# shenweichen/DeepCTR

Hardware: NVIDIA H100
Metric: samples/sec fwd+bwd DeepFM Criteo-synth (higher is better)
Workload: dtype f32

## Files before the change

deepctr_b200/_lib.py:

```python
import ctypes as C
import os
import subprocess

_HERE = os.path.dirname(os.path.abspath(__file__))
LIB_PATH = os.path.join(_HERE, "libb2ctr.so")
CSRC = os.path.join(_HERE, "csrc")

OK, ERR_INVALID_ARG, ERR_CUDA, ERR_UNSUPPORTED, ERR_WORKSPACE = 0, -1, -2, -3, -4
IDX_I32, IDX_I64 = 0, 1
POOL_NONE, POOL_SUM, POOL_MEAN, POOL_MAX = 0, 1, 2, 3
MASK_NONE, MASK_ZERO_ID, MASK_LENGTH = 0, 1, 2
HASH_NONE, HASH_FARM, HASH_FARM_MASK_ZERO = 0, 1, 2
WEIGHT_NONE, WEIGHT_RAW, WEIGHT_SOFTMAX = 0, 1, 2
ACT_NONE, ACT_RELU, ACT_SIGMOID, ACT_TANH = 0, 1, 2, 3
GEMM_FP32, GEMM_BF16X3 = 0, 1
TASK_BINARY, TASK_REGRESSION = 0, 1
MAX_FEATURES = 128
UNIFORM_STORE_GRADS = 1

ACT_BY_NAME = {None: ACT_NONE, "linear": ACT_NONE, "relu": ACT_RELU, "sigmoid": ACT_SIGMOID,
               "tanh": ACT_TANH}
POOL_BY_NAME = {"sum": POOL_SUM, "mean": POOL_MEAN, "max": POOL_MAX}


# ... 50 lines not shown
                ("dk", C.c_void_p), ("lddk", C.c_int64), ("dv", C.c_void_p), ("lddv", C.c_int64)]


_vp, _i32, _i64, _f32, _sz, _u64 = C.c_void_p, C.c_int32, C.c_int64, C.c_float, C.c_size_t, C.c_uint64

SIGNATURES = {
    "b2ctr_abi_version": (_i32, []),
    "b2ctr_last_error": (C.c_char_p, []),
    "b2ctr_launch_count": (_i64, []),
    "b2ctr_reset_launch_count": (None, []),
    "b2ctr_embed_gather_fwd": (_i32, [C.POINTER(Feature), _i32, _i64, _vp]),
    "b2ctr_embed_scatter_add": (_i32, [C.POINTER(Feature), _i32, _i64, _f32, _vp]),
    "b2ctr_embed_gather_uniform_fwd": (_i32, [C.POINTER(UniformGather), _i64, _vp]),
    "b2ctr_embed_scatter_uniform_bwd": (_i32, [C.POINTER(UniformGather), _vp, _vp, _vp, _f32, _f32,
                                               _i64, _vp]),
    "b2ctr_embed_oob_count": (_i32, [C.POINTER(C.c_int64), _i32, _vp]),
    "b2ctr_embed_update_sorted_workspace_bytes": (_sz, [_i32, _i32, _i64]),
    "b2ctr_embed_update_sorted": (_i32, [C.POINTER(UniformGather), _vp, _vp, _vp, _i32, _f32, _f32, _f32,
                                         C.POINTER(C.c_void_p), C.POINTER(C.c_void_p), _i64, _vp, _sz, _vp]),
    "b2ctr_hash64": (_i32, [_vp, _i32, _i64, _i64, _i32, _vp, _vp]),
    "b2ctr_init_normal": (_i32, [_vp, _i64, _f32, _f32, _u64, _vp]),
    "b2ctr_gemm_workspace_bytes": (_sz, [C.POINTER(Gemm)]),
    "b2ctr_enable_peer_access": (_i32, [_i32]),
    "b2ctr_host_pack": (_i32, [C.POINTER(C.c_void_p), C.POINTER(C.c_int64), C.POINTER(C.c_int64), _i32, _vp, _i32]),
    "b2ctr_gemm": (_i32, [C.POINTER(Gemm), _vp, _sz, _vp]),
    "b2ctr_planes_bytes": (_sz, [_i64, _i64]),
    "b2ctr_split_planes": (_i32, [_vp, _i64, _i64, _i64, _vp, _vp]),
    "b2ctr_bias_act_bwd_workspace_bytes": (_sz, [_i64, _i64]),
    "b2ctr_bias_act_bwd": (_i32, [_vp, _vp, _vp, _vp, _i64, _i64, _i64, _i32, _vp, _sz, _vp]),
    "b2ctr_bias_act_bwd_planes": (_i32, [_vp, _vp, _vp, _vp, _vp, _i64, _i64, _i64, _i32, _vp, _sz, _vp]),
# ... 157 lines not shown
```

deepctr_b200/csrc/common.cuh:

```cuda
#pragma once
#include <cuda_runtime.h>
#include <stdint.h>
#include <stdio.h>
#include <atomic>
#include "../../include/b2ctr.h"

namespace b2ctr {

void set_error(const char* fmt, ...);
extern std::atomic<long long> g_launches;
inline void count_launch(int n = 1) { g_launches.fetch_add(n, std::memory_order_relaxed); }

#define B2_REQUIRE(cond, ...)                         \
  do {                                                \
    if (!(cond)) {                                    \
      b2ctr::set_error(__VA_ARGS__);                  \
      return B2CTR_ERR_INVALID_ARG;                   \
    }                                                 \
  } while (0)

#define B2_CHECK_LAUNCH(name)                                                         \
  do {                                                                                \
    cudaError_t e__ = cudaGetLastError();                                             \
    if (e__ != cudaSuccess) {                                                         \
// ... 8 lines not shown
unsigned long long* oob_counter();

static inline int64_t ceil_div(int64_t a, int64_t b) { return (a + b - 1) / b; }

static inline int grid_for(int64_t work_items, int items_per_block, int blocks_per_sm) {
  int64_t need = ceil_div(work_items, items_per_block);
  int64_t cap = (int64_t)kNumSMs * blocks_per_sm;
  if (need < 1) need = 1;
  return (int)(need < cap ? need : cap);
}

static inline int64_t planes_rows_pad(int64_t rows) { return (rows + 255) / 256 * 256; }
static inline int64_t planes_cols_pad(int64_t cols) { return cols <= 64 ? 64 : (cols + 127) / 128 * 128; }

#ifdef __CUDACC__

__device__ __forceinline__ float4 ldg_stream_f4(const float* p) {
  float4 r;
  asm volatile("ld.global.nc.L1::no_allocate.v4.f32 {%0,%1,%2,%3}, [%4];"
               : "=f"(r.x), "=f"(r.y), "=f"(r.z), "=f"(r.w)
               : "l"(p));
  return r;
}
__device__ __forceinline__ float ldg_stream_f1(const float* p) {
  float r;
  asm volatile("ld.global.nc.L1::no_allocate.f32 %0, [%1];" : "=f"(r) : "l"(p));
  return r;
}
__device__ __forceinline__ void stg_stream_f4(float* p, float4 v) {
  asm volatile("st.global.L1::no_allocate.v4.f32 [%0], {%1,%2,%3,%4};" ::"l"(p), "f"(v.x),
// ... 91 lines not shown
```

deepctr_b200/csrc/embed.cu:

```cuda
#include "common.cuh"

namespace b2ctr {

namespace farm {
__host__ __device__ constexpr uint64_t k0() { return 0xc3a5c85c97cb3127ULL; }
__host__ __device__ constexpr uint64_t k1() { return 0xb492b66fbe98f273ULL; }
__host__ __device__ constexpr uint64_t k2() { return 0x9ae16a3b2f90404fULL; }
__device__ __forceinline__ uint64_t rot(uint64_t v, int s) { return (v >> s) | (v << (64 - s)); }
__device__ __forceinline__ uint64_t shift_mix(uint64_t v) { return v ^ (v >> 47); }
__device__ __forceinline__ uint64_t fetch64(const unsigned char* p) {
  uint64_t r = 0;
#pragma unroll
  for (int i = 7; i >= 0; --i) r = (r << 8) | p[i];
  return r;
}
__device__ __forceinline__ uint64_t fetch32(const unsigned char* p) {
  return (uint64_t)p[0] | ((uint64_t)p[1] << 8) | ((uint64_t)p[2] << 16) | ((uint64_t)p[3] << 24);
}
__device__ __forceinline__ uint64_t hash_len16(uint64_t u, uint64_t v, uint64_t mul) {
  uint64_t a = (u ^ v) * mul;
  a ^= (a >> 47);
  uint64_t b = (v ^ a) * mul;
  b ^= (b >> 47);
  b *= mul;
// ... 342 lines not shown
  float* fm;
  int64_t ldx;
  int64_t dense_ld;
  int64_t x_cols;
  uint64_t fm_mask;
  int32_t nfeat;
  int32_t ndense;
  int32_t dim;
  int32_t idx_dtype;
  int32_t has_lin;
  int32_t store_grads;
  float* const* peer_tab;
  float* const* peer_lin;
  int32_t world;
  int32_t wshift;
};

__device__ __forceinline__ float4 ld_peer_f4(const float* p) {
  float4 r;
  asm volatile("ld.global.L1::no_allocate.v4.f32 {%0,%1,%2,%3}, [%4];"
               : "=f"(r.x), "=f"(r.y), "=f"(r.z), "=f"(r.w)
               : "l"(p));
  return r;
}
__device__ __forceinline__ float ld_peer_f1(const float* p) {
  float r;
  asm volatile("ld.global.L1::no_allocate.f32 %0, [%1];" : "=f"(r) : "l"(p));
  return r;
}
__device__ __forceinline__ void red_peer_f4(float* p, float4 v) {
  asm volatile("red.relaxed.sys.global.add.v4.f32 [%0], {%1,%2,%3,%4};" ::"l"(p), "f"(v.x), "f"(v.y), "f"(v.z),
               "f"(v.w)
               : "memory");
}
__device__ __forceinline__ void red_peer_f1(float* p, float v) {
  asm volatile("red.relaxed.sys.global.add.f32 [%0], %1;" ::"l"(p), "f"(v) : "memory");
}
__device__ __forceinline__ float* shard_row(float* const* tabs, const UniParams& p, int f, int64_t id, int width) {
  const int64_t own = id & (int64_t)(p.world - 1);
  return tabs[(int64_t)f * p.world + own] + (id >> p.wshift) * width;
}

__device__ __forceinline__ int64_t uni_id(const UniParams& p, int f, int64_t b) {
  return load_idx(p.idx[f], b * p.idx_stride[f], p.idx_dtype);
}

template <int LPR, bool SHARD>
__global__ void __launch_bounds__(256, SHARD ? 3 : 4)
    gather_uniform_fwd_kernel(const __grid_constant__ UniParams p, int64_t batch) {
  constexpr int RPI = 32 / LPR;
  constexpr int U = 7;
  const int lane = threadIdx.x & 31;
  const int slot = lane / LPR, chunk = lane % LPR;
  const int F = p.nfeat, dim = p.dim;
  const uint64_t pol_keep = l2_policy_evict_last(), pol_stream = l2_policy_evict_first();
  const int64_t nwarps = (int64_t)gridDim.x * (blockDim.x >> 5);
  int64_t b = (int64_t)blockIdx.x * (blockDim.x >> 5) + (threadIdx.x >> 5);
  auto checked = [&](int f, int64_t bb) -> int64_t {
    if (bb >= batch || f >= F) return 0;
    const int64_t id = uni_id(p, f, bb);
    if (id_in_range(id, p.vocab[f])) return id;
    note_oob(p.oob);
    return -1;
// ... 19 lines not shown
        if (f < F) {
          if (id < 0) {
            v[u] = make_float4(0.f, 0.f, 0.f, 0.f);
          } else if (SHARD) {
            v[u] = ld_peer_f4(shard_row(p.peer_tab, p, f, id, dim) + chunk * 4);
          } else {
            v[u] = ldg_stream_f4_pol(p.table[f] + id * dim + chunk * 4, pol_stream);
          }
        }
      }
#pragma unroll
      for (int u = 0; u < U; ++u) {
        const int f = f0 + u * RPI + slot;
        if (f < F) {
          stg_stream_f4_pol(xrow + (int64_t)f * dim + chunk * 4, v[u], pol_stream);
          if ((p.fm_mask >> f) & 1ull) {
            s.x += v[u].x; s.y += v[u].y; s.z += v[u].z; s.w += v[u].w;
            q += v[u].x * v[u].x + v[u].y * v[u].y + v[u].z * v[u].z + v[u].w * v[u].w;
          }
        }
      }
    }
    if (p.fm != nullptr) {
#pragma unroll
      for (int o = LPR; o < 32; o <<= 1) {
        s.x += __shfl_xor_sync(0xffffffffu, s.x, o);
        s.y += __shfl_xor_sync(0xffffffffu, s.y, o);
        s.z += __shfl_xor_sync(0xffffffffu, s.z, o);
        s.w += __shfl_xor_sync(0xffffffffu, s.w, o);
      }
      float sq = slot == 0 ? (s.x * s.x + s.y * s.y + s.z * s.z + s.w * s.w) : 0.f;
      sq = warp_sum(sq);
      q = warp_sum(q);
      if (lane == 0) p.fm[b] = 0.5f * (sq - q);
    }
    if (p.linear != nullptr) {
      float l = 0.f;
      if (p.has_lin) {
        const bool ok0 = lane < F && id0 >= 0;
        const bool ok1 = lane + 32 < F && id1 >= 0;
        if (SHARD) {
          if (ok0) l += ld_peer_f1(shard_row(p.peer_lin, p, lane, id0, 1));
          if (ok1) l += ld_peer_f1(shard_row(p.peer_lin, p, lane + 32, id1, 1));
        } else {
          if (ok0) l += ldg_f1_pol(p.lin[lane] + id0, pol_keep);
          if (ok1) l += ldg_f1_pol(p.lin[lane + 32] + id1, pol_keep);
        }
      }
      l = warp_sum(l);
      if (lane == 0) p.linear[b] = l;
    }
    const int64_t c0 = (int64_t)F * dim;
    for (int64_t c = c0 + lane; c < p.x_cols; c += 32) {
      const int j = (int)(c - c0);
      xrow[c] = j < p.ndense ? p.dense[b * p.dense_ld + j] : 0.f;
    }
    id0 = nid0;
    id1 = nid1;
  }
}

template <int LPR, bool SHARD>
__global__ void __launch_bounds__(256, SHARD ? 2 : 3)
    scatter_uniform_bwd_kernel(const __grid_constant__ UniParams p, const float* __restrict__ dx,
                               const float* __restrict__ dfm, const float* __restrict__ dlinear,
                               float scale, float lin_scale, int64_t batch) {
  constexpr int RPI = 32 / LPR;
  constexpr int U = 4;
  const int lane = threadIdx.x & 31;
  const int slot = lane / LPR, chunk = lane % LPR;
  const int F = p.nfeat, dim = p.dim;
  const uint64_t pol_keep = l2_policy_evict_last(), pol_stream = l2_policy_evict_first();
  const int64_t nwarps = (int64_t)gridDim.x * (blockDim.x >> 5);
// ... 1 lines not shown
  auto checked = [&](int f, int64_t bb) -> int64_t {
    if (bb >= batch || f >= F) return 0;
    const int64_t id = uni_id(p, f, bb);
    return id_in_range(id, p.vocab[f]) ? id : -1;
  };
  int64_t id0 = checked(lane, b);
  int64_t id1 = checked(lane + 32, b);
  for (; b < batch; b += nwarps) {
    const int64_t bn = b + nwarps;
    const int64_t nid0 = checked(lane, bn);
    const int64_t nid1 = checked(lane + 32, bn);
    const float* xrow = p.x + b * p.ldx;
    const float* dxrow = dx ? dx + b * p.ldx : nullptr;
    const float gfm = dfm ? dfm[b] : 0.f;
    float4 s = make_float4(0.f, 0.f, 0.f, 0.f);
    if (dfm) {
      for (int f0 = 0; f0 < F; f0 += U * RPI) {
        float4 v[U];
#pragma unroll
        for (int u = 0; u < U; ++u) {
          const int f = f0 + u * RPI + slot;
          v[u] = make_float4(0.f, 0.f, 0.f, 0.f);
          if (f < F && ((p.fm_mask >> f) & 1ull))
            v[u] = *reinterpret_cast<const float4*>(xrow + (int64_t)f * dim + chunk * 4);
        }
#pragma unroll
        for (int u = 0; u < U; ++u) { s.x += v[u].x; s.y += v[u].y; s.z += v[u].z; s.w += v[u].w; }
      }
#pragma unroll
      for (int o = LPR; o < 32; o <<= 1) {
        s.x += __shfl_xor_sync(0xffffffffu, s.x, o);
// ... 194 lines not shown
  p->dense = g->dense;
  p->x = g->x;
  p->linear = g->linear;
  p->fm = g->fm;
  p->ldx = g->ldx;
  p->dense_ld = g->dense_ld;
  p->x_cols = g->x_cols > 0 ? g->x_cols : g->ldx;
  B2_REQUIRE(p->x_cols <= g->ldx && p->x_cols >= (int64_t)g->nfeat * dim + g->ndense, "uniform gather: x_cols out of range");
  p->fm_mask = g->fm_mask[0];
  p->nfeat = g->nfeat;
  p->ndense = g->ndense;
  p->dim = dim;
  p->idx_dtype = g->feats[0].idx_dtype;
  p->has_lin = g->world > 1 ? (g->peer_lin_tables != nullptr) : (g->lin_tables != nullptr);
  p->store_grads = (g->flags & B2CTR_UNIFORM_STORE_GRADS) ? 1 : 0;
  return B2CTR_OK;
}

}

using namespace b2ctr;

extern "C" {

b2ctr_status_t b2ctr_embed_gather_fwd(const b2ctr_feature_t* feats, int32_t nfeat, int64_t batch,
                                      void* stream) {
  bool vec4;
  int lanes;
  b2ctr_status_t s = validate_feats(feats, nfeat, batch, &vec4, &lanes);
  if (s != B2CTR_OK) return s;
  if (batch == 0) return B2CTR_OK;
// ... 31 lines not shown
#define B2_DISPATCH_LPR1(KERNEL, SH, dim, ...)                                 \
  switch ((dim) / 4) {                                                         \
    case 1: KERNEL<1, SH><<<grid, 256, 0, st>>>(__VA_ARGS__); break;           \
    case 2: KERNEL<2, SH><<<grid, 256, 0, st>>>(__VA_ARGS__); break;           \
    case 4: KERNEL<4, SH><<<grid, 256, 0, st>>>(__VA_ARGS__); break;           \
    case 8: KERNEL<8, SH><<<grid, 256, 0, st>>>(__VA_ARGS__); break;           \
    case 16: KERNEL<16, SH><<<grid, 256, 0, st>>>(__VA_ARGS__); break;         \
    default: KERNEL<32, SH><<<grid, 256, 0, st>>>(__VA_ARGS__); break;         \
  }
#define B2_DISPATCH_LPR(KERNEL, dim, ...)                                      \
  if (p.world > 1) { B2_DISPATCH_LPR1(KERNEL, true, dim, __VA_ARGS__) }        \
  else { B2_DISPATCH_LPR1(KERNEL, false, dim, __VA_ARGS__) }

b2ctr_status_t b2ctr_embed_gather_uniform_fwd(const b2ctr_uniform_gather_t* g, int64_t batch,
                                              void* stream) {
  UniParams p;
  b2ctr_status_t s = fill_uni(g, &p);
  if (s != B2CTR_OK) return s;
  if (batch <= 0) return B2CTR_OK;
  cudaStream_t st = (cudaStream_t)stream;
  const int grid = grid_for(batch, 8, 8);
  B2_DISPATCH_LPR(gather_uniform_fwd_kernel, p.dim, p, batch);
  B2_CHECK_LAUNCH("b2ctr_embed_gather_uniform_fwd");
  return B2CTR_OK;
}

b2ctr_status_t b2ctr_embed_scatter_uniform_bwd(const b2ctr_uniform_gather_t* g, const float* dx,
                                               const float* dfm, const float* dlinear, float scale,
                                               float lin_scale, int64_t batch, void* stream) {
  UniParams p;
  b2ctr_status_t s = fill_uni(g, &p);
  if (s != B2CTR_OK) return s;
  B2_REQUIRE(!dx || aligned16(dx), "uniform scatter: dx must be 16-byte aligned");
  if (batch <= 0) return B2CTR_OK;
  cudaStream_t st = (cudaStream_t)stream;
  const int grid = grid_for(batch, 8, 8);
  B2_DISPATCH_LPR(scatter_uniform_bwd_kernel, p.dim, p, dx, dfm, dlinear, scale, lin_scale, batch);
  B2_CHECK_LAUNCH("b2ctr_embed_scatter_uniform_bwd");
  return B2CTR_OK;
}

b2ctr_status_t b2ctr_hash64(const void* ids, int32_t idx_dtype, int64_t n, int64_t num_buckets,
                            int32_t mask_zero, int64_t* out, void* stream) {
  B2_REQUIRE(ids && out, "hash64: NULL pointer");
  B2_REQUIRE(idx_dtype == B2CTR_IDX_I32 || idx_dtype == B2CTR_IDX_I64, "hash64: bad idx_dtype");
  B2_REQUIRE(num_buckets >= (mask_zero ? 2 : 1), "hash64: num_buckets too small");
  if (n <= 0) return B2CTR_OK;
  hash64_kernel<<<grid_for(n, 256, 8), 256, 0, (cudaStream_t)stream>>>(ids, idx_dtype, n, num_buckets,
// ... 17 lines not shown
```

deepctr_b200/csrc/gemm_tc.cu:

```cuda
#include <cuda.h>
#include <cuda_bf16.h>
#include "common.cuh"

namespace b2ctr {

constexpr int kTM = 128;
constexpr int kTK = 64;
constexpr int kTcThreads = 256;

struct PlaneArgs {
  const __nv_bfloat16* a_hi; const __nv_bfloat16* a_lo;
  const __nv_bfloat16* b_hi; const __nv_bfloat16* b_lo;
  int64_t a_pitch, b_pitch;
  int a_mn, b_mn;
  float* c; const float* bias; float* ws;
  int64_t m, n, k_pad;
  int64_t ldc;
  int64_t k_per_split;
  float alpha;
  int act, accumulate, splits;
  const float* cin_t0; const float* cin_xk;
  int64_t cin_ld0, cin_ldk, cin_rows;
  int cin_m, cin_h, cin_hp, cin_on;
  float* fold_dt0; float* fold_dxk; int64_t fold_ldx;
// ... 166 lines not shown
        if (g.accumulate) v0 += cp[0];
        if (g.bias) v0 += g.bias[gn];
        cp[0] = act_apply(v0, g.act);
        if (two) {
          if (g.accumulate) v1 += cp[1];
          if (g.bias) v1 += g.bias[gn + 1];
          cp[1] = act_apply(v1, g.act);
        }
      }
    }
  }
}

__device__ __forceinline__ unsigned char* align1024(unsigned char* p) {
  return reinterpret_cast<unsigned char*>((reinterpret_cast<uintptr_t>(p) + 1023) & ~(uintptr_t)1023);
}

__device__ __forceinline__ uint32_t pack_bf16(__nv_bfloat16 lo, __nv_bfloat16 hi) {
  return (uint32_t)__bfloat16_as_ushort(lo) | ((uint32_t)__bfloat16_as_ushort(hi) << 16);
}

__global__ void tc_splitk_reduce_kernel(const PlaneArgs g) {
  const int64_t total = g.m * g.n;
  for (int64_t i = (int64_t)blockIdx.x * blockDim.x + threadIdx.x; i < total;
       i += (int64_t)gridDim.x * blockDim.x) {
    const int64_t gm = i / g.n, gn = i - gm * g.n;
    float v = 0.f;
    for (int z = 0; z < g.splits; ++z) v += g.ws[(int64_t)z * total + i];
    if (g.accumulate) v += g.c[gm * g.ldc + gn];
    if (g.bias) v += g.bias[gn];
    g.c[gm * g.ldc + gn] = act_apply(v, g.act);
  }
}
constexpr int kReduceBatch = 16;
// ... 1206 lines not shown
```

deepctr_b200/inputs.py:

```python
from collections import defaultdict, OrderedDict
from itertools import chain

import ctypes as C

import numpy as np
import torch

from . import _lib as L
from . import kernels as K
from . import engine as E
from .engine import Layer, l2


class Embedding(Layer):
    def __init__(self, input_dim, output_dim, embeddings_initializer=None, embeddings_regularizer=None,
                 mask_zero=False, name=None, **kwargs):
        Layer.__init__(self, name=name, **kwargs)
        self.input_dim, self.output_dim = int(input_dim), int(output_dim)
        self.embeddings_initializer = embeddings_initializer or E.RandomNormal(0.0, 0.05)
        self.embeddings_regularizer = embeddings_regularizer
        self.mask_zero = mask_zero
        self.supports_masking = mask_zero
        self.embeddings = self.add_weight("embeddings", (self.input_dim, self.output_dim),
                                          self.embeddings_initializer, self.embeddings_regularizer,
# ... 177 lines not shown
                 "mask_zero")


class EmbeddingPlanner(object):
    def __init__(self, model):
        from .layers.utils import Hash
        from .layers.sequence import SequencePoolingLayer, WeightedSequenceLayer
        self.model = model
        self.slots = []
        self.results = {}
        self.optimizer = None
        self.mode = "auto"
        self.fm_hint = None
        self.lin_hint = False
        self.tail_hint = None
        self.fm_result = None
        self.lin_result = None
        self._plans = {}
        consumers = defaultdict(list)
        for node in model._order:
            for t in E._flatten(node.inputs):
                consumers[id(t)].append(node)
        out_ids = set(id(t) for t in E._flatten(model.outputs))
        input_names = set(t.name for t in model.inputs)

        def as_input(t):
            return t.name if (isinstance(t.node.layer, E.InputLayer) and t.name in input_names) else None

        for node in model._order:
            if not isinstance(node.layer, Embedding) or not isinstance(node.inputs, E.KTensor):
# ... 205 lines not shown
        return len(self.main) == self.fast_n and not self.seq and (not self.lin or self._lin_matches_fast())

    def _lin_matches_fast(self):
        if not self.lin or len(self.lin) != self.fast_n or len(self.main) != self.fast_n:
            return False
        for a, b in zip(self.lin, self.main):
            if (a.input_name != b.input_name or a.maxlen != 1 or a.pool != L.POOL_NONE
                    or a.hash[0] != L.HASH_NONE):
                return False
        return True

    def begin_step(self, feed, training):
        self.results = {}
        self.fm_result = self.lin_result = None
        self.tail_done = None
        if not self.slots:
            return
        some = feed[self.slots[0].input_name].data
        batch, dev = some.shape[0], some.device
        grad = training and E.current_tape() is not None
        bufs = {}
        if self.main:
            bufs["main"] = E.Var(torch.empty((batch, self.main_ld), dtype=torch.float32, device=dev),
                                 ncols=self.main_width, owner=self)
        lin_fused = self.fast and self.lin_hint and self._lin_matches_fast()
        if self.lin and not lin_fused:
            bufs["lin"] = E.Var(torch.empty((batch, self.lin_ld), dtype=torch.float32, device=dev),
                                ncols=self.lin_width, owner=self)
        generic = []
        for s in self.slots:
# ... 40 lines not shown
                    self.tail_done = (c0, nd)
            linear = torch.empty((batch,), dtype=torch.float32, device=dev) if lin_fused else None
            fm, fm_mask = None, 0
            if self.fm_hint is not None:
                c0, nc = self.fm_hint
                d = fast_slots[0].dim
                if c0 % d == 0 and nc % d == 0 and c0 + nc <= self.fast_n * d:
                    fm = torch.empty((batch,), dtype=torch.float32, device=dev)
                    for f in range(c0 // d, (c0 + nc) // d):
                        fm_mask |= 1 << f
            plan = K.UniformPlan(feats, lin_tabs, dense, x, linear, fm, fm_mask)
            plan.g.x_cols = (self.main_ld if only_fast and not self.pnn_cols
                             else self.fast_n * fast_slots[0].dim)
            if peer is not None:
                plan.set_peers(self.dist.world, peer[0].table, peer[1].table if peer[1] is not None else None)
            K.embed_gather_uniform_fwd(plan, batch)
            if fm is not None:
                self.fm_result = (self.fm_hint, E.Var(fm.reshape(batch, 1)))
            if linear is not None:
                self.lin_result = E.Var(linear.reshape(batch, 1))
        if generic:
            feats = []
            for s in generic:
                buf = bufs[id(s)] if s.buf == "seq" else bufs[s.buf]
                feats.append(self._feature(s, feed, buf.data, buf.data.stride(0)))
            K.embed_gather_fwd(feats, batch)
        from . import ops
        vlin = E.Var(None, owner=self, name="__virtual_lin__")
        for s in self.slots:
            if s.buf == "lin" and lin_fused:
# ... 57 lines not shown
                st, tabs, ltabs, dimf = self.route
                dev = main.data.device
                grows = torch.empty((st["n_send"], dimf), dtype=torch.float32, device=dev)
                glin = torch.empty((st["n_send"],), dtype=torch.float32, device=dev) if lin_fused else None
                if dlin is None and glin is not None:
                    K.fill(glin, 0.0)
                pos = st["pos"]
                feats = [K.make_feature(grows, pos[:, f], main.data, out_col=s.col, out_ld=self.main_ld)
                         for f, s in enumerate(fast_slots)]
                bplan = K.UniformPlan(feats, [glin] * len(fast_slots) if lin_fused else None, None, main.data,
                                      None, None, plan.g.fm_mask[0])
                bplan.g.x_cols = plan.g.x_cols
                bplan.g.flags = L.UNIFORM_STORE_GRADS
                K.embed_scatter_uniform_bwd(bplan, dx, None if dfm is None else dfm.reshape(-1).contiguous(),
                                            None if dlin is None else dlin.reshape(-1).contiguous(),
                                            1.0, 1.0, batch)
                lr = opt["optimizer"].lr if opt and opt.get("optimizer") else 0.0
                sc = -lr / self.dist.world
                self.exchange.push(st, tabs, ltabs, dimf, grows, glin, sc, sc)
            elif (dx is not None or dfm is not None or dlin is not None) and plan.g.world > 1:
                from . import parallel
                emb, lin, token = self.peers
                parallel.device_barrier(self.dist, token)
                lr = opt["optimizer"].lr if opt and opt.get("optimizer") else 0.0
                sc = -lr / self.dist.world
                feats = [self._feature(s, feed, main.data, self.main_ld) for s in fast_slots]
                bplan = K.UniformPlan(feats, None, None, main.data, None, None, plan.g.fm_mask[0])
                bplan.g.x_cols = plan.g.x_cols
                bplan.set_peers(self.dist.world, emb.table, lin.table if (lin is not None and lin_fused) else None)
                K.embed_scatter_uniform_bwd(bplan, dx, None if dfm is None else dfm.reshape(-1).contiguous(),
                                            None if dlin is None else dlin.reshape(-1).contiguous(),
                                            sc, sc, batch)
            elif dx is not None or dfm is not None or dlin is not None:
                tgts = [self._target(s.emb.embeddings, opt) for s in fast_slots]
                feats = [self._feature(s, feed, main.data, self.main_ld, table=tgt)
                         for s, (tgt, _) in zip(fast_slots, tgts)]
                scale = max(abs(sc) for _, sc in tgts) * (-1.0 if any(sc < 0 for _, sc in tgts) else 1.0)
                lin_tabs, lin_scale = None, 0.0
                if lin_fused:
                    lt = [self._target(s.emb.embeddings, opt) for s in self.lin]
                    lin_tabs = [t.reshape(-1) for t, _ in lt]
                    lin_scale = max(abs(sc) for _, sc in lt) * (-1.0 if any(sc < 0 for _, sc in lt) else 1.0)
                bplan = K.UniformPlan(feats, lin_tabs, None, main.data, None, None, plan.g.fm_mask[0])
                bplan.g.x_cols = plan.g.x_cols
                if getattr(self, "sorted_update", False) and all(sc < 0 for _, sc in tgts):
                    o = opt["optimizer"]
                    adagrad = o.name == "adagrad"
                    acc = lacc = None
                    if adagrad:
                        acc = [self._adagrad_state(s.emb.embeddings) for s in fast_slots]
                        lacc = [self._adagrad_state(s.emb.embeddings).reshape(-1) for s in self.lin] if lin_fused else None
                    K.embed_update_sorted(bplan, dx, None if dfm is None else dfm.reshape(-1).contiguous(),
                                          None if dlin is None else dlin.reshape(-1).contiguous(),
                                          1 if adagrad else 0, o.lr, o.lr, 1e-7, acc, lacc, batch)
                    return self._backward_generic(feed, bufs, generic, opt, batch)
                K.embed_scatter_uniform_bwd(bplan, dx, None if dfm is None else dfm.reshape(-1).contiguous(),
                                            None if dlin is None else dlin.reshape(-1).contiguous(),
                                            scale, lin_scale, batch)
        self._backward_generic(feed, bufs, generic, opt, batch)

    @staticmethod
    def _adagrad_state(w):
        acc = w.opt_state.get("acc")
        if acc is None:
            acc = w.opt_state["acc"] = torch.empty_like(w.data)
            K.fill(acc, 0.1)
        return acc

    def _backward_generic(self, feed, bufs, generic, opt, batch):
        feats, scales = [], []
        flat = {}
        for s in generic:
            if not s.emb.embeddings.trainable:
# ... 17 lines not shown
        for sc in sorted(set(scales)):
            K.embed_scatter_add([f for f, s_ in zip(feats, scales) if s_ == sc], batch, sc)
        for (rows, sc), fs in flat.items():
            K.embed_scatter_add(fs, rows, sc)

    def lookup_fm(self, x):
        if x.base is None or x.base.owner is not self or x.ncols == -1:
            return None
        if x.base.ncols != self.main_width or x.base.data is None or x.base.data.shape[1] != self.main_ld:
            return None
        key = (x.col0, x.ncols)
        if self.fm_result is not None and self.fm_result[0] == key:
            return self.fm_result[1]
        if self.fast:
            self.fm_hint = key
        return None

    def lookup_rowsum(self, x):
        if x.base is None or x.base.owner is not self:
            return None
        if x.base.name == "__virtual_lin__":
            if x.col0 == 0 and x.ncols == self.lin_width and self.lin_result is not None:
                return self.lin_result
            raise L.B2ctrError("the linear-term lookups were fused into a row-sum but a layer asked for the rows")
        if (self.fast and x.base.ncols == self.lin_width and x.col0 == 0 and x.ncols == self.lin_width
                and x.base.data.shape[1] == self.lin_ld and self._lin_matches_fast()):
            self.lin_hint = True
        return None

    def dnn_input_place(self, layer):
# ... 581 lines not shown
```

deepctr_b200/kernels.py:

```python
import ctypes as C

import torch

from . import _lib as L

_workspace = {}
_retired = []


def _require_cuda(*tensors):
    for t in tensors:
        if t is not None and not t.is_cuda:
            raise L.B2ctrError("b2ctr kernels need CUDA tensors: there is no CPU fallback")


def stream():
    return C.c_void_p(torch.cuda.current_stream().cuda_stream)


def ptr(t):
    return C.c_void_p(t.data_ptr()) if t is not None else C.c_void_p(0)


def workspace(nbytes, device):
# ... 76 lines not shown
        self.g = L.UniformGather()
        self.g.feats = self.feat_arr
        if lin_tables is not None:
            self.lin_arr = (C.c_void_p * len(feats))(*[t.data_ptr() for t in lin_tables])
            self.g.lin_tables = self.lin_arr
        self.g.dense = dense.data_ptr() if dense is not None else None
        self.g.x = x.data_ptr()
        self.g.linear = linear.data_ptr() if linear is not None else None
        self.g.fm = fm.data_ptr() if fm is not None else None
        self.g.ldx = x.stride(0)
        self.g.dense_ld = dense.stride(0) if dense is not None else 0
        self.g.nfeat = len(feats)
        self.g.ndense = dense.shape[1] if dense is not None else 0
        self.g.fm_mask[0] = fm_mask & 0xFFFFFFFFFFFFFFFF
        self.g.fm_mask[1] = 0

    def set_peers(self, world, peer_tables, peer_lin_tables):
        self.peer_refs = (peer_tables, peer_lin_tables)
        self.g.world = world
        self.g.peer_tables = peer_tables.data_ptr()
        self.g.peer_lin_tables = peer_lin_tables.data_ptr() if peer_lin_tables is not None else None


def embed_gather_uniform_fwd(plan, batch):
    L.check(L.lib().b2ctr_embed_gather_uniform_fwd(C.byref(plan.g), batch, stream()),
            "embed_gather_uniform_fwd")


def embed_scatter_uniform_bwd(plan, dx, dfm, dlinear, scale, lin_scale, batch):
    L.check(L.lib().b2ctr_embed_scatter_uniform_bwd(C.byref(plan.g), ptr(dx), ptr(dfm), ptr(dlinear),
                                                    scale, lin_scale, batch, stream()),
            "embed_scatter_uniform_bwd")


def embed_update_sorted(plan, dx, dfm, dlinear, optimizer, lr, lin_lr, eps, acc_tables, lin_acc_tables, batch):
    nf = plan.g.nfeat
    dim = plan.feat_arr[0].dim
    nbytes = L.lib().b2ctr_embed_update_sorted_workspace_bytes(nf, dim, batch)
    dev = dx.device if dx is not None else (dfm.device if dfm is not None else dlinear.device)
    ws = workspace(nbytes, dev)
    acc = (C.c_void_p * nf)(*[t.data_ptr() for t in acc_tables]) if acc_tables is not None else None
    lacc = (C.c_void_p * nf)(*[t.data_ptr() for t in lin_acc_tables]) if lin_acc_tables is not None else None
    L.check(L.lib().b2ctr_embed_update_sorted(C.byref(plan.g), ptr(dx), ptr(dfm), ptr(dlinear), optimizer, lr, lin_lr,
                                              eps, acc, lacc, batch, ptr(ws), nbytes, stream()),
            "embed_update_sorted")

# ... 895 lines not shown
```

deepctr_b200/ops.py:

```python
import numpy as np
import torch

from . import _lib as L
from . import kernels as K
from . import engine as E

GEMM_PRECISION = L.GEMM_BF16X3


UNCAPTURABLE = 0


def mark_uncapturable():
    global UNCAPTURABLE
    UNCAPTURABLE += 1


def set_gemm_precision(mode):
    global GEMM_PRECISION
    GEMM_PRECISION = {"fp32": L.GEMM_FP32, "bf16x3": L.GEMM_BF16X3}[mode]


def _empty(shape, like):
    return torch.empty(shape, dtype=torch.float32, device=like.device)
# ... 7 lines not shown
        return int(max(1, min(592 // blocks, kred // 256)))
    tiles = ((m_out + 255) // 256) * ((n_out + 255) // 256)
    return int(max(1, min(74 // tiles if tiles <= 74 else 1, kred // 1024)))


def _as2d(x):
    t2, ld = x.as2d()
    if t2 is None:
        t = E.contiguous(x)
        t2 = t.reshape(-1, t.shape[-1])
        ld = t2.stride(0)
    return t2, ld


def _planes_of(var, t2):
    key = (t2.data_ptr(), tuple(t2.shape), t2.stride(0))
    if var.planes is None or var.planes[0] != key:
        var.planes = (key, K.split_planes(t2))
    return var.planes[1]


def dense(x, w, b=None, activation=None):
    act = L.ACT_BY_NAME.get(activation, None)
    fused_act = act if act is not None else L.ACT_NONE
    x2, _ = _as2d(x)
    m, kdim = x2.shape
    n = w.shape[1]
    wd = w.materialize() if isinstance(w, E.Weight) else w.data
    bd = (b.materialize() if isinstance(b, E.Weight) else b.data) if b is not None else None
    prec = GEMM_PRECISION if min(n, kdim) >= 16 else L.GEMM_FP32
# ... 1289 lines not shown
```

include/b2ctr.h:

```cpp
#ifndef B2CTR_H_
#define B2CTR_H_

#include <stddef.h>
#include <stdint.h>

#ifdef __cplusplus
extern "C" {
#endif

#if defined(_WIN32)
#define B2CTR_API
#else
#define B2CTR_API __attribute__((visibility("default")))
#endif

typedef int32_t b2ctr_status_t;
enum {
  B2CTR_OK = 0,
  B2CTR_ERR_INVALID_ARG = -1,
  B2CTR_ERR_CUDA = -2,
  B2CTR_ERR_UNSUPPORTED = -3,
  B2CTR_ERR_WORKSPACE = -4
};

// ... 60 lines not shown
  int64_t ldx;
  int64_t dense_ld;
  int64_t x_cols;
  int32_t nfeat;
  int32_t ndense;
  uint64_t fm_mask[2];
  int32_t flags;
  int32_t world;
  float* const* peer_tables;
  float* const* peer_lin_tables;
} b2ctr_uniform_gather_t;
#define B2CTR_UNIFORM_STORE_GRADS 1

B2CTR_API b2ctr_status_t b2ctr_embed_gather_uniform_fwd(const b2ctr_uniform_gather_t* g,
                                                       int64_t batch, void* stream);

B2CTR_API b2ctr_status_t b2ctr_embed_scatter_uniform_bwd(const b2ctr_uniform_gather_t* g,
                                                        const float* dx, const float* dfm,
                                                        const float* dlinear, float scale,
                                                        float lin_scale, int64_t batch,
                                                        void* stream);

B2CTR_API b2ctr_status_t b2ctr_embed_oob_count(int64_t* count, int32_t reset, void* stream);

B2CTR_API size_t b2ctr_embed_update_sorted_workspace_bytes(int32_t nfeat, int32_t dim, int64_t batch);
B2CTR_API b2ctr_status_t b2ctr_embed_update_sorted(const b2ctr_uniform_gather_t* g, const float* dx,
                                                  const float* dfm, const float* dlinear, int32_t optimizer,
                                                  float lr, float lin_lr, float eps, float* const* acc_tables,
                                                  float* const* lin_acc_tables, int64_t batch, void* workspace,
                                                  size_t workspace_bytes, void* stream);

B2CTR_API b2ctr_status_t b2ctr_hash64(const void* ids, int32_t idx_dtype, int64_t n,
                                     int64_t num_buckets, int32_t mask_zero, int64_t* out,
                                     void* stream);

B2CTR_API b2ctr_status_t b2ctr_init_normal(float* dst, int64_t n, float mean, float std,
// ... 340 lines not shown
```

Before: 34.84 million.

## Fuse bf16x3 plane split and FM sum caching into embedding gather kernel

The forward embedding gather kernel now also writes the hi/lo bf16 planes of the concatenated embedding matrix, so the first dense layer's bf16x3 GEMM can skip a separate split_planes pass. It also stores the per-sample FM field sum so the backward scatter can reuse it instead of re-gathering all embeddings. The cost is extra stores and zero-padding in the gather kernel, a lower occupancy bound (3 blocks/SM), and a hint mechanism that only activates after the first step has recorded the expected width.

```diff
diff --git a/deepctr_b200/_lib.py b/deepctr_b200/_lib.py
--- a/deepctr_b200/_lib.py
+++ b/deepctr_b200/_lib.py
@@ -88,6 +88,9 @@
     "b2ctr_embed_gather_uniform_fwd": (_i32, [C.POINTER(UniformGather), _i64, _vp]),
     "b2ctr_embed_scatter_uniform_bwd": (_i32, [C.POINTER(UniformGather), _vp, _vp, _vp, _f32, _f32,
                                                _i64, _vp]),
+    "b2ctr_embed_gather_uniform_fwd_ex": (_i32, [C.POINTER(UniformGather), _vp, _vp, _i64, _i64, _vp]),
+    "b2ctr_embed_scatter_uniform_bwd_ex": (_i32, [C.POINTER(UniformGather), _vp, _vp, _vp, _vp, _f32, _f32,
+                                                  _i64, _vp]),
     "b2ctr_embed_oob_count": (_i32, [C.POINTER(C.c_int64), _i32, _vp]),
     "b2ctr_embed_update_sorted_workspace_bytes": (_sz, [_i32, _i32, _i64]),
     "b2ctr_embed_update_sorted": (_i32, [C.POINTER(UniformGather), _vp, _vp, _vp, _i32, _f32, _f32, _f32,
diff --git a/deepctr_b200/csrc/common.cuh b/deepctr_b200/csrc/common.cuh
--- a/deepctr_b200/csrc/common.cuh
+++ b/deepctr_b200/csrc/common.cuh
@@ -1,5 +1,6 @@
 #pragma once
 #include <cuda_runtime.h>
+#include <cuda_bf16.h>
 #include <stdint.h>
 #include <stdio.h>
 #include <atomic>
@@ -46,6 +47,9 @@
 static inline int64_t planes_cols_pad(int64_t cols) { return cols <= 64 ? 64 : (cols + 127) / 128 * 128; }
 
 #ifdef __CUDACC__
+__device__ __forceinline__ uint32_t pack_bf16(__nv_bfloat16 lo, __nv_bfloat16 hi) {
+  return (uint32_t)__bfloat16_as_ushort(lo) | ((uint32_t)__bfloat16_as_ushort(hi) << 16);
+}
 
 __device__ __forceinline__ float4 ldg_stream_f4(const float* p) {
   float4 r;
diff --git a/deepctr_b200/csrc/embed.cu b/deepctr_b200/csrc/embed.cu
--- a/deepctr_b200/csrc/embed.cu
+++ b/deepctr_b200/csrc/embed.cu
@@ -380,7 +380,24 @@
   float* const* peer_lin;
   int32_t world;
   int32_t wshift;
+  float* fm_sum;
+  __nv_bfloat16* xp_hi;
+  __nv_bfloat16* xp_lo;
+  int64_t xp_pitch;
+  int64_t xp_rows_pad;
 };
+
+__device__ __forceinline__ void store_planes4(const UniParams& p, int64_t off, float4 v) {
+  const __nv_bfloat16 h0 = __float2bfloat16_rn(v.x), h1 = __float2bfloat16_rn(v.y);
+  const __nv_bfloat16 h2 = __float2bfloat16_rn(v.z), h3 = __float2bfloat16_rn(v.w);
+  uint2 h, l;
+  h.x = pack_bf16(h0, h1);
+  h.y = pack_bf16(h2, h3);
+  l.x = pack_bf16(__float2bfloat16_rn(v.x - __bfloat162float(h0)), __float2bfloat16_rn(v.y - __bfloat162float(h1)));
+  l.y = pack_bf16(__float2bfloat16_rn(v.z - __bfloat162float(h2)), __float2bfloat16_rn(v.w - __bfloat162float(h3)));
+  *reinterpret_cast<uint2*>(p.xp_hi + off) = h;
+  *reinterpret_cast<uint2*>(p.xp_lo + off) = l;
+}
 
 __device__ __forceinline__ float4 ld_peer_f4(const float* p) {
   float4 r;
@@ -411,8 +428,8 @@
   return load_idx(p.idx[f], b * p.idx_stride[f], p.idx_dtype);
 }
 
-template <int LPR, bool SHARD>
-__global__ void __launch_bounds__(256, SHARD ? 3 : 4)
+template <int LPR, bool SHARD, bool EXTRA>
+__global__ void __launch_bounds__(256, (SHARD || EXTRA) ? 3 : 4)
     gather_uniform_fwd_kernel(const __grid_constant__ UniParams p, int64_t batch) {
   constexpr int RPI = 32 / LPR;
   constexpr int U = 7;
@@ -462,6 +479,7 @@
         const int f = f0 + u * RPI + slot;
         if (f < F) {
           stg_stream_f4_pol(xrow + (int64_t)f * dim + chunk * 4, v[u], pol_stream);
+          if (EXTRA && p.xp_hi) store_planes4(p, b * p.xp_pitch + (int64_t)f * dim + chunk * 4, v[u]);
           if ((p.fm_mask >> f) & 1ull) {
             s.x += v[u].x; s.y += v[u].y; s.z += v[u].z; s.w += v[u].w;
             q += v[u].x * v[u].x + v[u].y * v[u].y + v[u].z * v[u].z + v[u].w * v[u].w;
@@ -477,6 +495,7 @@
         s.z += __shfl_xor_sync(0xffffffffu, s.z, o);
         s.w += __shfl_xor_sync(0xffffffffu, s.w, o);
       }
+      if (EXTRA && p.fm_sum != nullptr && slot == 0) *reinterpret_cast<float4*>(p.fm_sum + b * dim + chunk * 4) = s;
       float sq = slot == 0 ? (s.x * s.x + s.y * s.y + s.z * s.z + s.w * s.w) : 0.f;
       sq = warp_sum(sq);
       q = warp_sum(q);
@@ -503,8 +522,25 @@
       const int j = (int)(c - c0);
       xrow[c] = j < p.ndense ? p.dense[b * p.dense_ld + j] : 0.f;
     }
+    if (EXTRA && p.xp_hi) {
+      for (int64_t c = c0 + lane; c < p.xp_pitch; c += 32) {
+        const int j = (int)(c - c0);
+        const float v = j < p.ndense ? p.dense[b * p.dense_ld + j] : 0.f;
+        const __nv_bfloat16 h = __float2bfloat16_rn(v);
+        p.xp_hi[b * p.xp_pitch + c] = h;
+        p.xp_lo[b * p.xp_pitch + c] = __float2bfloat16_rn(v - __bfloat162float(h));
+      }
+    }
     id0 = nid0;
     id1 = nid1;
+  }
+  if (EXTRA && p.xp_hi) {
+    const uint4 z = make_uint4(0u, 0u, 0u, 0u);
+    for (int64_t r = b; r < p.xp_rows_pad; r += nwarps)
+      for (int64_t c = lane * 8; c < p.xp_pitch; c += 256) {
+        *reinterpret_cast<uint4*>(p.xp_hi + r * p.xp_pitch + c) = z;
+        *reinterpret_cast<uint4*>(p.xp_lo + r * p.xp_pitch + c) = z;
+      }
   }
 }
 
@@ -536,7 +572,9 @@
     const float* dxrow = dx ? dx + b * p.ldx : nullptr;
     const float gfm = dfm ? dfm[b] : 0.f;
     float4 s = make_float4(0.f, 0.f, 0.f, 0.f);
-    if (dfm) {
+    if (dfm && p.fm_sum) {
+      s = *reinterpret_cast<const float4*>(p.fm_sum + b * dim + chunk * 4);
+    } else if (dfm) {
       for (int f0 = 0; f0 < F; f0 += U * RPI) {
         float4 v[U];
 #pragma unroll
@@ -761,7 +799,22 @@
   p->idx_dtype = g->feats[0].idx_dtype;
   p->has_lin = g->world > 1 ? (g->peer_lin_tables != nullptr) : (g->lin_tables != nullptr);
   p->store_grads = (g->flags & B2CTR_UNIFORM_STORE_GRADS) ? 1 : 0;
+  p->fm_sum = nullptr;
+  p->xp_hi = p->xp_lo = nullptr;
+  p->xp_pitch = p->xp_rows_pad = 0;
   return B2CTR_OK;
+}
+
+template <bool SHARD, bool EXTRA>
+static void launch_gather(const UniParams& p, int64_t batch, int grid, cudaStream_t st) {
+  switch (p.dim / 4) {
+    case 1: gather_uniform_fwd_kernel<1, SHARD, EXTRA><<<grid, 256, 0, st>>>(p, batch); break;
+    case 2: gather_uniform_fwd_kernel<2, SHARD, EXTRA><<<grid, 256, 0, st>>>(p, batch); break;
+    case 4: gather_uniform_fwd_kernel<4, SHARD, EXTRA><<<grid, 256, 0, st>>>(p, batch); break;
+    case 8: gather_uniform_fwd_kernel<8, SHARD, EXTRA><<<grid, 256, 0, st>>>(p, batch); break;
+    case 16: gather_uniform_fwd_kernel<16, SHARD, EXTRA><<<grid, 256, 0, st>>>(p, batch); break;
+    default: gather_uniform_fwd_kernel<32, SHARD, EXTRA><<<grid, 256, 0, st>>>(p, batch); break;
+  }
 }
 
 }
@@ -823,13 +876,36 @@
 
 b2ctr_status_t b2ctr_embed_gather_uniform_fwd(const b2ctr_uniform_gather_t* g, int64_t batch,
                                               void* stream) {
+  return b2ctr_embed_gather_uniform_fwd_ex(g, nullptr, nullptr, 0, batch, stream);
+}
+
+b2ctr_status_t b2ctr_embed_gather_uniform_fwd_ex(const b2ctr_uniform_gather_t* g, float* fm_sum, void* x_planes,
+                                                 int64_t x_planes_cols, int64_t batch, void* stream) {
   UniParams p;
   b2ctr_status_t s = fill_uni(g, &p);
   if (s != B2CTR_OK) return s;
+  B2_REQUIRE(!fm_sum || (g->fm && aligned16(fm_sum)), "uniform gather: fm_sum needs fm and 16-byte alignment");
+  p.fm_sum = fm_sum;
+  if (x_planes) {
+    B2_REQUIRE(x_planes_cols >= (int64_t)g->nfeat * p.dim + g->ndense && x_planes_cols <= p.x_cols,
+               "uniform gather: x_planes_cols must be in [F*dim + ndense, x_cols]");
+    B2_REQUIRE(aligned16(x_planes), "uniform gather: x_planes must be 16-byte aligned");
+    p.xp_pitch = planes_cols_pad(x_planes_cols);
+    p.xp_rows_pad = planes_rows_pad(batch);
+    p.xp_hi = (__nv_bfloat16*)x_planes;
+    p.xp_lo = p.xp_hi + p.xp_rows_pad * p.xp_pitch;
+  }
   if (batch <= 0) return B2CTR_OK;
   cudaStream_t st = (cudaStream_t)stream;
-  const int grid = grid_for(batch, 8, 8);
-  B2_DISPATCH_LPR(gather_uniform_fwd_kernel, p.dim, p, batch);
+  if (p.fm_sum || p.xp_hi) {
+    const int grid = grid_for(batch, 8, 3);
+    if (p.world > 1) launch_gather<true, true>(p, batch, grid, st);
+    else launch_gather<false, true>(p, batch, grid, st);
+  } else {
+    const int grid = grid_for(batch, 8, 8);
+    if (p.world > 1) launch_gather<true, false>(p, batch, grid, st);
+    else launch_gather<false, false>(p, batch, grid, st);
+  }
   B2_CHECK_LAUNCH("b2ctr_embed_gather_uniform_fwd");
   return B2CTR_OK;
 }
@@ -837,10 +913,18 @@
 b2ctr_status_t b2ctr_embed_scatter_uniform_bwd(const b2ctr_uniform_gather_t* g, const float* dx,
                                                const float* dfm, const float* dlinear, float scale,
                                                float lin_scale, int64_t batch, void* stream) {
+  return b2ctr_embed_scatter_uniform_bwd_ex(g, dx, dfm, nullptr, dlinear, scale, lin_scale, batch, stream);
+}
+
+b2ctr_status_t b2ctr_embed_scatter_uniform_bwd_ex(const b2ctr_uniform_gather_t* g, const float* dx,
+                                                  const float* dfm, const float* fm_sum, const float* dlinear,
+                                                  float scale, float lin_scale, int64_t batch, void* stream) {
   UniParams p;
   b2ctr_status_t s = fill_uni(g, &p);
   if (s != B2CTR_OK) return s;
   B2_REQUIRE(!dx || aligned16(dx), "uniform scatter: dx must be 16-byte aligned");
+  B2_REQUIRE(!fm_sum || aligned16(fm_sum), "uniform scatter: fm_sum must be 16-byte aligned");
+  p.fm_sum = const_cast<float*>(fm_sum);
   if (batch <= 0) return B2CTR_OK;
   cudaStream_t st = (cudaStream_t)stream;
   const int grid = grid_for(batch, 8, 8);
diff --git a/deepctr_b200/csrc/gemm_tc.cu b/deepctr_b200/csrc/gemm_tc.cu
--- a/deepctr_b200/csrc/gemm_tc.cu
+++ b/deepctr_b200/csrc/gemm_tc.cu
@@ -204,10 +204,6 @@
 
 __device__ __forceinline__ unsigned char* align1024(unsigned char* p) {
   return reinterpret_cast<unsigned char*>((reinterpret_cast<uintptr_t>(p) + 1023) & ~(uintptr_t)1023);
-}
-
-__device__ __forceinline__ uint32_t pack_bf16(__nv_bfloat16 lo, __nv_bfloat16 hi) {
-  return (uint32_t)__bfloat16_as_ushort(lo) | ((uint32_t)__bfloat16_as_ushort(hi) << 16);
 }
 
 __global__ void tc_splitk_reduce_kernel(const PlaneArgs g) {
diff --git a/deepctr_b200/inputs.py b/deepctr_b200/inputs.py
--- a/deepctr_b200/inputs.py
+++ b/deepctr_b200/inputs.py
@@ -215,6 +215,7 @@
         self.fm_hint = None
         self.lin_hint = False
         self.tail_hint = None
+        self.planes_hint = None
         self.fm_result = None
         self.lin_result = None
         self._plans = {}
@@ -450,6 +451,7 @@
         self.results = {}
         self.fm_result = self.lin_result = None
         self.tail_done = None
+        self.planes_result = None
         if not self.slots:
             return
         some = feed[self.slots[0].input_name].data
@@ -520,6 +522,11 @@
                              else self.fast_n * fast_slots[0].dim)
             if peer is not None:
                 plan.set_peers(self.dist.world, peer[0].table, peer[1].table if peer[1] is not None else None)
+            from . import ops
+            kd = self.main_width + (self.tail_done[1] if self.tail_done is not None else 0)
+            if (self.planes_hint == kd and only_fast and not self.pnn_cols and batch >= 128
+                    and ops.GEMM_PRECISION == L.GEMM_BF16X3):
+                self.planes_result = (kd, plan.set_planes(kd))
             K.embed_gather_uniform_fwd(plan, batch)
             if fm is not None:
                 self.fm_result = (self.fm_hint, E.Var(fm.reshape(batch, 1)))
@@ -607,7 +614,7 @@
                 bplan.g.flags = L.UNIFORM_STORE_GRADS
                 K.embed_scatter_uniform_bwd(bplan, dx, None if dfm is None else dfm.reshape(-1).contiguous(),
                                             None if dlin is None else dlin.reshape(-1).contiguous(),
-                                            1.0, 1.0, batch)
+                                            1.0, 1.0, batch, fm_sum=plan.fm_sum)
                 lr = opt["optimizer"].lr if opt and opt.get("optimizer") else 0.0
                 sc = -lr / self.dist.world
                 self.exchange.push(st, tabs, ltabs, dimf, grows, glin, sc, sc)
@@ -623,7 +630,7 @@
                 bplan.set_peers(self.dist.world, emb.table, lin.table if (lin is not None and lin_fused) else None)
                 K.embed_scatter_uniform_bwd(bplan, dx, None if dfm is None else dfm.reshape(-1).contiguous(),
                                             None if dlin is None else dlin.reshape(-1).contiguous(),
-                                            sc, sc, batch)
+                                            sc, sc, batch, fm_sum=plan.fm_sum)
             elif dx is not None or dfm is not None or dlin is not None:
                 tgts = [self._target(s.emb.embeddings, opt) for s in fast_slots]
                 feats = [self._feature(s, feed, main.data, self.main_ld, table=tgt)
@@ -649,7 +656,7 @@
                     return self._backward_generic(feed, bufs, generic, opt, batch)
                 K.embed_scatter_uniform_bwd(bplan, dx, None if dfm is None else dfm.reshape(-1).contiguous(),
                                             None if dlin is None else dlin.reshape(-1).contiguous(),
-                                            scale, lin_scale, batch)
+                                            scale, lin_scale, batch, fm_sum=plan.fm_sum)
         self._backward_generic(feed, bufs, generic, opt, batch)
 
     @staticmethod
@@ -697,6 +704,17 @@
             return self.fm_result[1]
         if self.fast:
             self.fm_hint = key
+        return None
+
+    def lookup_planes(self, x, t2):
+        base = x.base
+        if (x.col0 != 0 or x.ncols == -1 or base.data is None or base.ncols != self.main_width
+                or t2.data_ptr() != base.data.data_ptr() or t2.stride(0) != base.data.stride(0)):
+            return None
+        if self.planes_result is not None and self.planes_result[0] == t2.shape[1]:
+            return self.planes_result[1]
+        if self.fast:
+            self.planes_hint = t2.shape[1]
         return None
 
     def lookup_rowsum(self, x):
diff --git a/deepctr_b200/kernels.py b/deepctr_b200/kernels.py
--- a/deepctr_b200/kernels.py
+++ b/deepctr_b200/kernels.py
@@ -114,6 +114,16 @@
         self.g.ndense = dense.shape[1] if dense is not None else 0
         self.g.fm_mask[0] = fm_mask & 0xFFFFFFFFFFFFFFFF
         self.g.fm_mask[1] = 0
+        self.fm_sum = (torch.empty((x.shape[0], feats[0].dim), dtype=torch.float32, device=x.device)
+                       if fm is not None else None)
+        self.x_rows, self.x_device = x.shape[0], x.device
+        self.x_planes, self.x_planes_cols = None, 0
+
+    def set_planes(self, cols):
+        nbytes = L.lib().b2ctr_planes_bytes(self.x_rows, cols)
+        self.x_planes = torch.empty((nbytes,), dtype=torch.uint8, device=self.x_device)
+        self.x_planes_cols = cols
+        return self.x_planes
 
     def set_peers(self, world, peer_tables, peer_lin_tables):
         self.peer_refs = (peer_tables, peer_lin_tables)
@@ -123,13 +133,14 @@
 
 
 def embed_gather_uniform_fwd(plan, batch):
-    L.check(L.lib().b2ctr_embed_gather_uniform_fwd(C.byref(plan.g), batch, stream()),
+    L.check(L.lib().b2ctr_embed_gather_uniform_fwd_ex(C.byref(plan.g), ptr(plan.fm_sum), ptr(plan.x_planes),
+                                                      plan.x_planes_cols, batch, stream()),
             "embed_gather_uniform_fwd")
 
 
-def embed_scatter_uniform_bwd(plan, dx, dfm, dlinear, scale, lin_scale, batch):
-    L.check(L.lib().b2ctr_embed_scatter_uniform_bwd(C.byref(plan.g), ptr(dx), ptr(dfm), ptr(dlinear),
-                                                    scale, lin_scale, batch, stream()),
+def embed_scatter_uniform_bwd(plan, dx, dfm, dlinear, scale, lin_scale, batch, fm_sum=None):
+    L.check(L.lib().b2ctr_embed_scatter_uniform_bwd_ex(C.byref(plan.g), ptr(dx), ptr(dfm), ptr(fm_sum),
+                                                       ptr(dlinear), scale, lin_scale, batch, stream()),
             "embed_scatter_uniform_bwd")
 
 
diff --git a/deepctr_b200/ops.py b/deepctr_b200/ops.py
--- a/deepctr_b200/ops.py
+++ b/deepctr_b200/ops.py
@@ -45,6 +45,11 @@
 
 
 def _planes_of(var, t2):
+    base = var.base
+    if base is not None and hasattr(base.owner, "lookup_planes"):
+        planes = base.owner.lookup_planes(var, t2)
+        if planes is not None:
+            return planes
     key = (t2.data_ptr(), tuple(t2.shape), t2.stride(0))
     if var.planes is None or var.planes[0] != key:
         var.planes = (key, K.split_planes(t2))
diff --git a/include/b2ctr.h b/include/b2ctr.h
--- a/include/b2ctr.h
+++ b/include/b2ctr.h
@@ -98,12 +98,20 @@
 
 B2CTR_API b2ctr_status_t b2ctr_embed_gather_uniform_fwd(const b2ctr_uniform_gather_t* g,
                                                        int64_t batch, void* stream);
+B2CTR_API b2ctr_status_t b2ctr_embed_gather_uniform_fwd_ex(const b2ctr_uniform_gather_t* g, float* fm_sum,
+                                                          void* x_planes, int64_t x_planes_cols, int64_t batch,
+                                                          void* stream);
 
 B2CTR_API b2ctr_status_t b2ctr_embed_scatter_uniform_bwd(const b2ctr_uniform_gather_t* g,
                                                         const float* dx, const float* dfm,
                                                         const float* dlinear, float scale,
                                                         float lin_scale, int64_t batch,
                                                         void* stream);
+B2CTR_API b2ctr_status_t b2ctr_embed_scatter_uniform_bwd_ex(const b2ctr_uniform_gather_t* g,
+                                                           const float* dx, const float* dfm,
+                                                           const float* fm_sum, const float* dlinear,
+                                                           float scale, float lin_scale, int64_t batch,
+                                                           void* stream);
 
 B2CTR_API b2ctr_status_t b2ctr_embed_oob_count(int64_t* count, int32_t reset, void* stream);
 
```

Measured after the change: 35.89 million (median of 6 runs). 1.03x the previous value.
